# amorim-cleison/sign-language-nlp

Measured on AMD Instinct MI355X. Metric: train seq/s (batch=50,len=48), higher is better.
Workload: dtype bf16x3; 1 GPU; cfg2: Transformer train step E512 H8 N6 F512 batch 50 len 48 |src| 3000 |tgt| 202 dropout 0.1, fwd+CE+bwd+clip(0.5)+SGD(m=.9); launch=eager stream launches (auto: timed both in 9 untimed pre-warmup steps + warmup), per_gpu=independent fit (grid shard)

## Files before the change

### sign-language-nlp_amd/csrc/common.hpp

```cpp
#pragma once
#include <vector>
#include <hip/hip_runtime.h>
#include <atomic>
#include <mutex>
#include <stdint.h>
#include <stdio.h>
#include <string.h>

#include "../../include/slnlp.h"

namespace slnlp {

void set_error(const char* fmt, ...);

#define SLNLP_CHECK_ARG(cond, ...)                 \
    do {                                           \
        if (!(cond)) {                             \
            ::slnlp::set_error(__VA_ARGS__);       \
            return SLNLP_ERR_INVALID_ARG;          \
        }                                          \
    } while (0)

#define SLNLP_CHECK_LAUNCH(what)                                              \
    do {                                                                      \
        hipError_t e__ = hipGetLastError();                                   \
        if (e__ != hipSuccess) {                                              \
            ::slnlp::set_error("%s: %s", what, hipGetErrorString(e__));       \
            return SLNLP_ERR_LAUNCH;                                          \
        }                                                                     \
    } while (0)

#define SLNLP_TRY(expr)            \
    do {                           \
        int rc__ = (expr);         \
        if (rc__ != 0) return rc__; \
    } while (0)

static inline int ceil_div(long a, long b) { return (int)((a + b - 1) / b); }

struct DeviceOnce {
    std::mutex mu;
    std::atomic<bool> done[64];
    DeviceOnce() { for (auto& d : done) d.store(false, std::memory_order_relaxed); }
    template <class F>
    int run(F&& init) {
        int dev = 0;
        if (hipGetDevice(&dev) != hipSuccess || dev < 0 || dev >= 64) dev = 0;
        if (done[dev].load(std::memory_order_acquire)) return 0;
        std::lock_guard<std::mutex> lk(mu);
        if (done[dev].load(std::memory_order_relaxed)) return 0;
        const int rc = init();
        if (rc == 0) done[dev].store(true, std::memory_order_release);
        return rc;
    }
};

#ifndef SLNLP_PROBE_FENCES
#define SLNLP_PROBE_FENCES 0
#endif
__device__ __forceinline__ void probe_kernel_begin() {
#if SLNLP_PROBE_FENCES & 1
    __builtin_amdgcn_fence(__ATOMIC_ACQUIRE, "agent");
    asm volatile("s_waitcnt vmcnt(0)" ::: "memory");
#endif
}
__device__ __forceinline__ void probe_kernel_end() {
#if SLNLP_PROBE_FENCES & 2
    asm volatile("s_waitcnt vmcnt(0)" ::: "memory");
    __builtin_amdgcn_fence(__ATOMIC_RELEASE, "agent");
    asm volatile("s_waitcnt vmcnt(0)" ::: "memory");
#endif
}

__device__ __forceinline__ void gather_id_rows(const int64_t* __restrict__ X, const int64_t* __restrict__ order, long first, int B, int S,
                                               int64_t* __restrict__ out) {
    const int lane = threadIdx.x & 63;
    const int wave = __builtin_amdgcn_readfirstlane((int)(blockIdx.x * 4 + (threadIdx.x >> 6)));
    const int nwaves = gridDim.x * 4;
    for (int r = wave; r < B; r += nwaves) {
        const int64_t* src = X + (order ? order[r] : first + r) * S;
        int64_t* dst = out + (long)r * S;
        for (int c = lane; c < S; c += 64) dst[c] = src[c];
    }
}
static inline int gather_rows_grid(int B) { return B >= 256 ? 64 : (B + 3) / 4; }

template <class Row = long, class Count, class F>
__device__ __forceinline__ void wave_rows(Count n, F f) {
    const int lane = threadIdx.x & 63;
    const int wave = __builtin_amdgcn_readfirstlane((int)(blockIdx.x * 4 + (threadIdx.x >> 6)));
    const int nwaves = gridDim.x * 4;
    for (Row r = wave; r < n; r += nwaves) f(r, lane);
}
constexpr int WAVE_ROWS_MAX_BLOCKS = 2048;
static inline int wave_rows_grid(int64_t n) { return (int)((n + 3) / 4 < WAVE_ROWS_MAX_BLOCKS ? (n + 3) / 4 : WAVE_ROWS_MAX_BLOCKS); }
__device__ __forceinline__ int lanes_below(unsigned long long ballot) {
    return (int)__builtin_amdgcn_mbcnt_hi((unsigned)(ballot >> 32), __builtin_amdgcn_mbcnt_lo((unsigned)ballot, 0u));
}

struct RngState {
    unsigned long long seed;
    unsigned long long step;
};

struct DropKey { unsigned ks[5]; };
__device__ __forceinline__ DropKey dropout_key(const unsigned long long* rng, int site) {
    const unsigned long long k = rng[0] + 0x9E3779B97F4A7C15ull * rng[1];
    DropKey K;
    K.ks[0] = (unsigned)k; K.ks[1] = (unsigned)(k >> 32); K.ks[2] = (unsigned)site; K.ks[3] = 0u;
    K.ks[4] = 0x1BD11BDAu ^ K.ks[0] ^ K.ks[1] ^ K.ks[2] ^ K.ks[3];
    return K;
}

#ifndef SLNLP_THREEFRY_ROUNDS
#define SLNLP_THREEFRY_ROUNDS 12
#endif
__device__ __forceinline__ uint4 threefry4x32(unsigned c0, unsigned c1, const DropKey& K) {
    constexpr int ROT[8][2] = {{10, 26}, {11, 21}, {13, 27}, {23, 5}, {6, 20}, {17, 11}, {25, 10}, {18, 20}};
    unsigned x0 = c0 + K.ks[0], x1 = c1 + K.ks[1], x2 = K.ks[2], x3 = K.ks[3];
#pragma unroll
    for (int r = 0; r < SLNLP_THREEFRY_ROUNDS; ++r) {
        if ((r & 1) == 0) {
            x0 += x1; x1 = __builtin_rotateleft32(x1, ROT[r & 7][0]) ^ x0;
            x2 += x3; x3 = __builtin_rotateleft32(x3, ROT[r & 7][1]) ^ x2;
        } else {
            x0 += x3; x3 = __builtin_rotateleft32(x3, ROT[r & 7][0]) ^ x0;
            x2 += x1; x1 = __builtin_rotateleft32(x1, ROT[r & 7][1]) ^ x2;
        }
        if ((r & 3) == 3) {
            const int s = (r + 1) >> 2;
            x0 += K.ks[s % 5]; x1 += K.ks[(s + 1) % 5]; x2 += K.ks[(s + 2) % 5]; x3 += K.ks[(s + 3) % 5] + (unsigned)s;
        }
    }
    return make_uint4(x0, x1, x2, x3);
}

constexpr unsigned SEED_STAGE_BOOTSTRAP = SLNLP_BOOT_STAGE;
struct SeedKey { unsigned ks[5]; unsigned epoch; };
__device__ __forceinline__ SeedKey seed_key(unsigned long long seed, unsigned epoch) {
    SeedKey K;
    K.ks[0] = (unsigned)seed; K.ks[1] = (unsigned)(seed >> 32); K.ks[2] = 0u; K.ks[3] = 0u;
    K.ks[4] = 0x1BD11BDAu ^ K.ks[0] ^ K.ks[1];
    K.epoch = epoch;
    return K;
}
__device__ __forceinline__ uint4 seed_words(unsigned index, unsigned word2, const SeedKey& K) {
    constexpr int ROT[8][2] = {{10, 26}, {11, 21}, {13, 27}, {23, 5}, {6, 20}, {17, 11}, {25, 10}, {18, 20}};
    unsigned x0 = index + K.ks[0], x1 = K.epoch + K.ks[1], x2 = word2 + K.ks[2], x3 = K.ks[3];
#pragma unroll
    for (int r = 0; r < SLNLP_THREEFRY_ROUNDS; ++r) {
        if ((r & 1) == 0) {
            x0 += x1; x1 = __builtin_rotateleft32(x1, ROT[r & 7][0]) ^ x0;
            x2 += x3; x3 = __builtin_rotateleft32(x3, ROT[r & 7][1]) ^ x2;
        } else {
            x0 += x3; x3 = __builtin_rotateleft32(x3, ROT[r & 7][0]) ^ x0;
            x2 += x1; x1 = __builtin_rotateleft32(x1, ROT[r & 7][1]) ^ x2;
        }
        if ((r & 3) == 3) {
            const int s = (r + 1) >> 2;
            x0 += K.ks[s % 5]; x1 += K.ks[(s + 1) % 5]; x2 += K.ks[(s + 2) % 5]; x3 += K.ks[(s + 3) % 5] + (unsigned)s;
        }
    }
    return make_uint4(x0, x1, x2, x3);
}

__device__ __forceinline__ unsigned drop_cc(unsigned c) { return ((c >> 5) << 4) | (c & 15u); }
__device__ __forceinline__ int drop_half(unsigned c) { return (int)((c >> 4) & 1u); }

__device__ __forceinline__ uint4 dropout_bits8(const DropKey& key, unsigned r4, unsigned cc) { return threefry4x32(cc, r4, key); }

__host__ __device__ __forceinline__ unsigned dropout_threshold(float p) {
    const double t = (double)p * 65536.0 + 0.5;
    return t >= 65535.0 ? 65535u : (unsigned)t;
}

__device__ __forceinline__ unsigned pick_lot(const uint4& v, int half, int r) {
    const unsigned long long lo = (unsigned long long)v.x | ((unsigned long long)v.y << 32);
    const unsigned long long hi = (unsigned long long)v.z | ((unsigned long long)v.w << 32);
    return (unsigned)((half ? hi : lo) >> (16 * (r & 3))) & 0xFFFFu;
}

__device__ __forceinline__ bool dropout_keep(const DropKey& key, unsigned r, unsigned c, unsigned thr) {
    const uint4 b = dropout_bits8(key, r >> 2, drop_cc(c));
    return pick_lot(b, drop_half(c), (int)(r & 3u)) >= thr;
}
__device__ __forceinline__ bool dropout_keep(const unsigned long long* rng, int site,
                                             unsigned r, unsigned c, unsigned thr) {
    return dropout_keep(dropout_key(rng, site), r, c, thr);
}

struct PlaneOut {
    unsigned short* hi = nullptr;
    unsigned short* lo = nullptr;
    unsigned char* q8 = nullptr;
};
__device__ __forceinline__ unsigned pack_fp8x4(float a, float b, float c, float d) {
    a = fminf(fmaxf(a, -448.f), 448.f); b = fminf(fmaxf(b, -448.f), 448.f);
    c = fminf(fmaxf(c, -448.f), 448.f); d = fminf(fmaxf(d, -448.f), 448.f);
    int w = __builtin_amdgcn_cvt_pk_fp8_f32(a, b, 0, false);
    w = __builtin_amdgcn_cvt_pk_fp8_f32(c, d, w, true);
    return (unsigned)w;
}
__device__ __forceinline__ void split_bf16(float x, unsigned short& h, unsigned short& l) {
    const __bf16 hb = (__bf16)x;
    h = __builtin_bit_cast(unsigned short, hb);
    const __bf16 b = (__bf16)(x - (float)hb);
    l = __builtin_bit_cast(unsigned short, b);
}
__device__ __forceinline__ unsigned short head_bf16(float x) { return __builtin_bit_cast(unsigned short, (__bf16)x); }
__device__ __forceinline__ void store_planes1(const PlaneOut& po, long idx, float v) {
    if (!po.hi) return;
    unsigned short h, l;
    split_bf16(v, h, l);
    po.hi[idx] = h;
    po.lo[idx] = l;
    if (po.q8) po.q8[idx] = (unsigned char)(pack_fp8x4(v, 0.f, 0.f, 0.f) & 0xFFu);
}
__device__ __forceinline__ void store_planes4(const PlaneOut& po, long idx, float4 v) {
    if (!po.hi) return;
    unsigned short h[4], l[4];
    split_bf16(v.x, h[0], l[0]); split_bf16(v.y, h[1], l[1]); split_bf16(v.z, h[2], l[2]); split_bf16(v.w, h[3], l[3]);
    uint2 w;
    w.x = h[0] | ((unsigned)h[1] << 16); w.y = h[2] | ((unsigned)h[3] << 16);
    *reinterpret_cast<uint2*>(po.hi + idx) = w;
    w.x = l[0] | ((unsigned)l[1] << 16); w.y = l[2] | ((unsigned)l[3] << 16);
    *reinterpret_cast<uint2*>(po.lo + idx) = w;
    if (po.q8) *reinterpret_cast<unsigned*>(po.q8 + idx) = pack_fp8x4(v.x, v.y, v.z, v.w);
}

template <int CTRL>
__device__ __forceinline__ float dpp_mov(float v) {
    return __builtin_bit_cast(float, __builtin_amdgcn_update_dpp(0, __builtin_bit_cast(int, v), CTRL, 0xF, 0xF, true));
}
constexpr int DPP_XOR1 = 0xB1, DPP_XOR2 = 0x4E;
constexpr int DPP_HALF_MIRROR = 0x141, DPP_MIRROR = 0x140;
__device__ __forceinline__ float lane_bcast(float v, int lane) {
    return __builtin_bit_cast(float, __builtin_amdgcn_readlane(__builtin_bit_cast(int, v), lane));
}
__device__ __forceinline__ float row16_sum(float v) {
    v += dpp_mov<DPP_XOR1>(v);
    v += dpp_mov<DPP_XOR2>(v);
    v += dpp_mov<DPP_HALF_MIRROR>(v);
    v += dpp_mov<DPP_MIRROR>(v);
    return v;
}
__device__ __forceinline__ float row16_max(float v) {
    v = fmaxf(v, dpp_mov<DPP_XOR1>(v));
    v = fmaxf(v, dpp_mov<DPP_XOR2>(v));
    v = fmaxf(v, dpp_mov<DPP_HALF_MIRROR>(v));
    v = fmaxf(v, dpp_mov<DPP_MIRROR>(v));
    return v;
}
__device__ __forceinline__ float wave_sum(float v) {
    v = row16_sum(v);
    return (lane_bcast(v, 0) + lane_bcast(v, 16)) + (lane_bcast(v, 32) + lane_bcast(v, 48));
}
__device__ __forceinline__ float wave_max(float v) {
    v = row16_max(v);
    return fmaxf(fmaxf(lane_bcast(v, 0), lane_bcast(v, 16)), fmaxf(lane_bcast(v, 32), lane_bcast(v, 48)));
}
template <int CTRL>
__device__ __forceinline__ double dpp_mov_d(double v) {
    const int lo = __builtin_amdgcn_update_dpp(0, __double2loint(v), CTRL, 0xF, 0xF, true);
    const int hi = __builtin_amdgcn_update_dpp(0, __double2hiint(v), CTRL, 0xF, 0xF, true);
    return __hiloint2double(hi, lo);
// ... 264 lines not shown
```

### sign-language-nlp_amd/csrc/gemm_planes.hip

```cpp
#include <algorithm>
#include <vector>

#include "common.hpp"
#include "gemm_jobs.hpp"

namespace slnlp {

typedef __attribute__((ext_vector_type(8))) __bf16 bf16x8;
typedef __attribute__((ext_vector_type(4))) short s16x4;
typedef __attribute__((ext_vector_type(8))) short s16x8;
typedef __attribute__((ext_vector_type(4))) float f32x4;
typedef __attribute__((address_space(3))) void* lds_vp;
typedef __attribute__((address_space(1))) const void* glb_vp;
typedef __attribute__((ext_vector_type(4))) unsigned int u32x4;

constexpr int PT = 64;
constexpr int PTHREADS = 512;

__device__ __forceinline__ int mswz(int k) { return (((k >> 1) & 1) | (((k >> 3) & 1) << 1)) << 1; }

template <bool KMAJOR>
__device__ __forceinline__ int img_off(int row, int k) {
    if (KMAJOR) return row * PT + ((((k >> 3) ^ (row & 7)) << 3) | (k & 7));
    return k * PT + ((((row >> 3) ^ mswz(k)) << 3) | (row & 7));
}

template <bool KMAJOR>
__device__ __forceinline__ unsigned plane_lane_off(long ld, int row0, int wave, int lane) {
    const int line = 8 * wave + (lane >> 3), ps = lane & 7;
    const long e = KMAJOR ? (long)(row0 + line) * ld + ((ps ^ (line & 7)) << 3) : (long)line * ld + row0 + ((ps ^ mswz(line)) << 3);
    return (unsigned)(e * 2);
}
__device__ __forceinline__ void dma_piece(const unsigned short* __restrict__ plane, long kterm, unsigned lane_off, unsigned short* dst) {
    const char* src = reinterpret_cast<const char*>(plane + kterm) + lane_off;
    __builtin_amdgcn_global_load_lds((glb_vp)src, (lds_vp)dst, 16, 0, 0);
}

template <bool KMAJOR>
__device__ __forceinline__ bf16x8 pfrag(const unsigned short* __restrict__ img, int r0, int kk, int lane) {
    if (KMAJOR) {
        return *reinterpret_cast<const bf16x8*>(img + img_off<true>(r0 + (lane & 15), kk * 32 + ((lane >> 4) << 3)));
    } else {
        const int i = lane & 15, kb = kk * 32 + ((lane >> 4) << 3) + (i >> 2), col = r0 + ((i & 3) << 2);
        typedef __attribute__((address_space(3))) s16x4* lds_p;
        const s16x4 v0 = __builtin_amdgcn_ds_read_tr16_b64_v4i16((lds_p)(img + img_off<false>(col, kb)));
        const s16x4 v1 = __builtin_amdgcn_ds_read_tr16_b64_v4i16((lds_p)(img + img_off<false>(col, kb + 4)));
        const s16x8 v = {v0[0], v0[1], v0[2], v0[3], v1[0], v1[1], v1[2], v1[3]};
        return __builtin_bit_cast(bf16x8, v);
    }
}

template <bool KMAJOR>
__device__ __forceinline__ int img32_off(int row, int k) {
    if (KMAJOR) {
        const int line = row >> 1, sl = ((row & 1) << 2) | (k >> 3);
        return line * PT + (((sl ^ (line & 7)) << 3) | (k & 7));
    }
    return img_off<false>(row, k);
}
template <bool KMAJOR>
__device__ __forceinline__ unsigned slab32_lane_off(long ld, int row0, int row_last, int wave, int lane) {
    const int h = wave >> 2, line = 8 * (wave & 3) + (lane >> 3), ps = lane & 7;
    const int r_img = min(row0 + PT * h, row_last);
    long e;
    if (KMAJOR) {
        const int sl = ps ^ (line & 7);
        e = (long)(r_img + 2 * line + (sl >> 2)) * ld + ((sl & 3) << 3);
    } else {
        e = (long)line * ld + r_img + ((ps ^ mswz(line)) << 3);
    }
    return (unsigned)(e * 2);
}
template <bool KMAJOR>
__device__ __forceinline__ bf16x8 pfrag32(const unsigned short* __restrict__ img, int r0, int lane) {
    if (KMAJOR) return *reinterpret_cast<const bf16x8*>(img + img32_off<true>(r0 + (lane & 15), (lane >> 4) << 3));
    return pfrag<false>(img, r0, 0, lane);
}

__device__ __forceinline__ float pbf2f(unsigned short h) { return __uint_as_float(((unsigned)h) << 16); }

__device__ __forceinline__ void st_agent2(float* p, float a, float b) {
    const unsigned long long v = (unsigned long long)__float_as_uint(a) | ((unsigned long long)__float_as_uint(b) << 32);
    __hip_atomic_store(reinterpret_cast<unsigned long long*>(p), v, __ATOMIC_RELAXED, __HIP_MEMORY_SCOPE_AGENT);
}
__device__ __forceinline__ float2 ld_agent2(const float* p) {
    const unsigned long long v = __hip_atomic_load(reinterpret_cast<const unsigned long long*>(p), __ATOMIC_RELAXED, __HIP_MEMORY_SCOPE_AGENT);
    return make_float2(__uint_as_float((unsigned)v), __uint_as_float((unsigned)(v >> 32)));
}

#if SLNLP_PROBE_FENCES == 128
constexpr int TS_MAX = 1 << 16;
constexpr int TS_W = 8;
__device__ unsigned long long g_ts[TS_MAX][TS_W];
__device__ unsigned g_ts_n;
#ifdef SLNLP_PROBE_EPI
#define TS_CLK(slot) do { } while (0)
#else
#define TS_CLK(slot) do { if (slot == 1) ts[6] = __builtin_amdgcn_s_memtime(); if (slot == 2) ts[7] = __builtin_amdgcn_s_memtime(); } while (0)
#endif
#define TS_MARK(slot) do { if (threadIdx.x == 0) { ts[slot] = __builtin_amdgcn_s_memrealtime(); \
        TS_CLK(slot); } } while (0)
#else
#define TS_MARK(slot) do { } while (0)
#endif
#if SLNLP_PROBE_FENCES == 128 && defined(SLNLP_PROBE_EPI)
#define TS_EPI(slot) do { if (threadIdx.x == 0) ts[slot] = __builtin_amdgcn_s_memrealtime(); } while (0)
#else
#define TS_EPI(slot) do { } while (0)
#endif

template <int BM, int BN>
struct WaveGrid {
    static constexpr int WN = BM % 64 == 0 ? 2 : 4, WM = 8 / WN, WN_SH = WN == 2 ? 1 : 2;
    static constexpr int MT = BM / WM / 16, NT = BN / WN / 16;
    static constexpr int SUBM = (BM + PT - 1) / PT;
    static_assert(BM % (16 * WM) == 0 && BN % (16 * WN) == 0, "whole MFMA tiles per wave");
    static __device__ __forceinline__ int wm0(int wave) { return (wave >> WN_SH) * (BM / WM); }
    static __device__ __forceinline__ int wn0(int wave) { return (wave & (WN - 1)) * (BN / WN); }
};

__device__ __forceinline__ unsigned plane_lane_off_clamped(long ld, int row0, int row_max, int wave, int lane) {
    const int line = 8 * wave + (lane >> 3), ps = lane & 7;
    return (unsigned)(((long)min(row0 + line, row_max) * ld + ((ps ^ (line & 7)) << 3)) * 2);
}

template <int NSPLIT, bool AK, bool BK, int BM, int BN, int BKS, int NST>
__device__ __forceinline__ void plane_kloop(const slnlp_gemm_args& g, unsigned short* smem, int bm0, int bn0, int kt0, int kt1,
                                            bool do_rowsum, f32x4 (&acc)[WaveGrid<BM, BN>::MT][WaveGrid<BM, BN>::NT],
                                            float (&rowsum)[WaveGrid<BM, BN>::SUBM], unsigned long long* ts) {
    constexpr int NPA = NSPLIT == 3 ? 2 : 1, NPB = NSPLIT >= 2 ? 2 : 1;
    using WG = WaveGrid<BM, BN>;
    constexpr int SUBM = WG::SUBM, SUBN = BN / PT;
    constexpr int MT = WG::MT, NT = WG::NT;
    constexpr int IMG_E = PT * BKS;
    constexpr int A_E = BM * BKS, B_E = BN * BKS;
    constexpr int A_LO = A_E, B_HI = NPA * A_E, B_LO = B_HI + B_E;
    constexpr int STAGE = NPA * A_E + NPB * B_E;
    constexpr bool HALF_A = BM % PT != 0;
    constexpr int PIECES = HALF_A ? NPA + 1 + NPB * SUBN : (NPA * SUBM + NPB * SUBN) * BKS / 64;
    constexpr int PIECES_HI = HALF_A && NPA == 1 ? PIECES - 1 : PIECES;
    static_assert(BKS == 64 || (BM % 128 == 0 && BN % 128 == 0), "32-k stages move 128-row slabs");
    static_assert(!HALF_A || (AK && BKS == 64 && BM == PT + PT / 2), "the 96-row panel is built for k-major A and 64-k stages");
    const int tid = threadIdx.x, lane = tid & 63, wave = __builtin_amdgcn_readfirstlane(tid >> 6);
    const int wm0 = WG::wm0(wave), wn0 = WG::wn0(wave);
    const int am_last = ((g.M + PT - 1) / PT - 1) * PT, bn_last = ((g.N + PT - 1) / PT - 1) * PT;

    constexpr int APC = HALF_A ? 1 : BKS == 64 ? SUBM : SUBM / 2, BPC = BKS == 64 ? SUBN : SUBN / 2;
    unsigned aoff[APC], boff[BPC];
    unsigned aoff_half = 0;
#pragma unroll
    for (int q = 0; q < APC; ++q) {
        if constexpr (HALF_A) aoff[q] = plane_lane_off_clamped(g.lda_p, bm0, am_last + PT - 1, wave, lane);
        else if constexpr (BKS == 64) aoff[q] = plane_lane_off<AK>(g.lda_p, BM > PT ? min(bm0 + q * PT, am_last) : bm0, wave, lane);
        else aoff[q] = slab32_lane_off<AK>(g.lda_p, bm0 + 2 * q * PT, am_last, wave, lane);
    }
    if constexpr (HALF_A) aoff_half = plane_lane_off_clamped(g.lda_p, bm0 + PT, am_last + PT - 1, wave & 3, lane);
#pragma unroll
    for (int q = 0; q < BPC; ++q) {
        if constexpr (BKS == 64) boff[q] = plane_lane_off<BK>(g.ldb_p, BN > PT ? min(bn0 + q * PT, bn_last) : bn0, wave, lane);
        else boff[q] = slab32_lane_off<BK>(g.ldb_p, bn0 + 2 * q * PT, bn_last, wave, lane);
    }
    constexpr int PSTEP = BKS == 64 ? 1 : 2;
    auto issue = [&](int kt, int stage) {
        const int k0 = (kt < kt1 ? kt : kt0) * BKS;
        const long ka = AK ? (long)k0 : (long)k0 * g.lda_p, kb = BK ? (long)k0 : (long)k0 * g.ldb_p;
        unsigned short* s = smem + stage * STAGE + wave * 512;
#pragma unroll
        for (int q = 0; q < APC; ++q) {
            dma_piece(g.A_hi, ka, aoff[q], s + q * PSTEP * IMG_E);
            if (NPA == 2) dma_piece(g.A_lo, ka, aoff[q], s + (A_LO + q * PSTEP * IMG_E));
        }
        if constexpr (HALF_A) {
            unsigned short* sh = smem + stage * STAGE + IMG_E + (wave & 3) * 512;
            if (wave < 4) dma_piece(g.A_hi, ka, aoff_half, sh);
            else if (NPA == 2) dma_piece(g.A_lo, ka, aoff_half, sh + A_LO);
        }
#pragma unroll
        for (int q = 0; q < BPC; ++q) {
            dma_piece(g.B_hi, kb, boff[q], s + (B_HI + q * PSTEP * IMG_E));
            if (NPB == 2) dma_piece(g.B_lo, kb, boff[q], s + (B_LO + q * PSTEP * IMG_E));
        }
    };

    for (int t = 0; t < NST - 1; ++t) issue(kt0 + t, t);
    for (int kt = kt0; kt < kt1; ++kt) {
        const int it = kt - kt0;
        if (PIECES_HI == PIECES || wave < 4) asm volatile("s_waitcnt vmcnt(%0)\n\ts_waitcnt lgkmcnt(0)" ::"n"((NST - 2) * PIECES) : "memory");
        else asm volatile("s_waitcnt vmcnt(%0)\n\ts_waitcnt lgkmcnt(0)" ::"n"((NST - 2) * PIECES_HI) : "memory");
        __builtin_amdgcn_s_barrier();
        asm volatile("" ::: "memory");
#if SLNLP_PROBE_FENCES == 128
        if (kt == kt0) TS_MARK(1);
#endif
        issue(kt + NST - 1, (it + NST - 1) % NST);
        const unsigned short* s = smem + (it % NST) * STAGE;
#pragma unroll
        for (int kk = 0; kk < BKS / 32; ++kk) {
            constexpr int JB = NT > 4 ? 4 : NT;
            bf16x8 ah[MT], al[MT];
#pragma unroll
            for (int i = 0; i < MT; ++i) {
                const int row = wm0 + 16 * i;
                if constexpr (BKS == 64) {
                    ah[i] = pfrag<AK>(s + (row / PT) * IMG_E, row % PT, kk, lane);
                    if (NPA == 2) al[i] = pfrag<AK>(s + (A_LO + (row / PT) * IMG_E), row % PT, kk, lane);
                } else {
                    ah[i] = pfrag32<AK>(s + (row / PT) * IMG_E, row % PT, lane);
                    if (NPA == 2) al[i] = pfrag32<AK>(s + (A_LO + (row / PT) * IMG_E), row % PT, lane);
                }
            }
#pragma unroll
            for (int j0 = 0; j0 < NT; j0 += JB) {
                bf16x8 bh[JB], bl[JB];
#pragma unroll
                for (int j = 0; j < JB; ++j) {
                    const int row = wn0 + 16 * (j0 + j);
                    if constexpr (BKS == 64) {
                        bh[j] = pfrag<BK>(s + (B_HI + (row / PT) * IMG_E), row % PT, kk, lane);
                        if (NPB == 2) bl[j] = pfrag<BK>(s + (B_LO + (row / PT) * IMG_E), row % PT, kk, lane);
                    } else {
                        bh[j] = pfrag32<BK>(s + (B_HI + (row / PT) * IMG_E), row % PT, lane);
                        if (NPB == 2) bl[j] = pfrag32<BK>(s + (B_LO + (row / PT) * IMG_E), row % PT, lane);
                    }
                }
#pragma unroll
                for (int i = 0; i < MT; ++i)
#pragma unroll
                    for (int j = 0; j < JB; ++j) {
                        f32x4& c = acc[i][j0 + j];
                        if (NPA == 2) c = __builtin_amdgcn_mfma_f32_16x16x32_bf16(al[i], bh[j], c, 0, 0, 0);
                        if (NPB == 2) c = __builtin_amdgcn_mfma_f32_16x16x32_bf16(ah[i], bl[j], c, 0, 0, 0);
                        c = __builtin_amdgcn_mfma_f32_16x16x32_bf16(ah[i], bh[j], c, 0, 0, 0);
                    }
            }
        }
        if (do_rowsum) {
            constexpr int OCT = BKS / 8;
            const int row = tid & 63, kq = ((tid >> 6) % OCT) * 8, sub0 = (tid >> 6) / OCT;
#pragma unroll
            for (int sm = 0; sm < SUBM; sm += 8 / OCT) {
                const int im = sm + sub0;
                if constexpr (HALF_A) {
                    if (im * PT + row >= BM) continue;
                }
                float t = 0.f;
#pragma unroll
                for (int k = 0; k < 8; ++k) {
                    const int off = BKS == 64 ? img_off<AK>(row, kq + k) : img32_off<AK>(row, kq + k);
                    t += pbf2f(s[im * IMG_E + off]);
                    if (NPA == 2) t += pbf2f(s[A_LO + im * IMG_E + off]);
                }
                if (BKS == 64) rowsum[sm] += t;
                else if (kt & 1) rowsum[sm + 1] += t;
                else rowsum[sm] += t;
            }
        }
    }
}

template <int NSPLIT, int BM, int BN, int BKS, int NST>
__device__ __forceinline__ void plane_tile(const PlaneJob& job, int lid, bool placed, unsigned short* smem) {
    unsigned long long* tsp = nullptr;
#if SLNLP_PROBE_FENCES == 128
    unsigned long long ts[TS_W] = {0, 0, 0, 0, 0, 0, 0, 0};
    struct TsFlush {
        unsigned long long* t;
        __device__ ~TsFlush() {
            if (threadIdx.x == 0) {
                t[4] = __builtin_amdgcn_s_memrealtime();
                unsigned hw;
                asm volatile("s_getreg_b32 %0, hwreg(HW_REG_XCC_ID)" : "=s"(hw));
                t[5] = ((unsigned long long)hw << 32) | blockIdx.x;
                const unsigned i = atomicAdd(&g_ts_n, 1u) & (unsigned)(TS_MAX - 1);
                for (int k = 0; k < TS_W; ++k) g_ts[i][k] = t[k];
            }
        }
    } ts_flush{ts};
    tsp = ts;
    TS_MARK(0);
#endif
    using WG = WaveGrid<BM, BN>;
    constexpr int SUBM = WG::SUBM;
    constexpr int MT = WG::MT, NT = WG::NT;
    constexpr int KSUB = PT / BKS;
    const slnlp_gemm_args& g = job.a;
    const int tid = threadIdx.x, lane = tid & 63, wave = __builtin_amdgcn_readfirstlane(tid >> 6);
    const int wm0 = WG::wm0(wave), wn0 = WG::wn0(wave);
    const int nks = job.nks;
    int bx, by, ks, tile;
    {
        const int nwg = job.tiles_x * job.tiles_y * nks;
        const int xcd = lid & 7, q = nwg >> 3, r = nwg & 7;
        const int t = placed ? lid : (xcd < r ? xcd * (q + 1) : r * (q + 1) + (xcd - r) * q) + (lid >> 3);
        const int ntiles = job.tiles_x * job.tiles_y;
        ks = t / ntiles;
        tile = t - ks * ntiles;
        constexpr int GR = BM >= 256 ? 2 : BM >= 128 ? 4 : 8;
        const int grp = tile / (GR * job.tiles_x), rem = tile - grp * (GR * job.tiles_x);
        const int rows_here = min(GR, job.tiles_y - grp * GR);
        bx = rem / rows_here;
        by = grp * GR + (rem - bx * rows_here);
        tile = by * job.tiles_x + bx;
    }
    const int bm0 = by * BM, bn0 = bx * BN;
    const int M = g.M, N = g.N, K = g.K;
    const int ktiles = (K + PT - 1) / PT;
    const int kt0 = (int)((long)ktiles * ks / nks) * KSUB, kt1 = (int)((long)ktiles * (ks + 1) / nks) * KSUB;

    f32x4 acc[MT][NT];
#pragma unroll
    for (int i = 0; i < MT; ++i)
#pragma unroll
        for (int j = 0; j < NT; ++j) acc[i][j] = f32x4{0.f, 0.f, 0.f, 0.f};
    const bool do_rowsum = (g.rowsum_a != nullptr) && (bx == 0);
    float rowsum[SUBM];
#pragma unroll
    for (int i = 0; i < SUBM; ++i) rowsum[i] = 0.f;

    if constexpr (BM % PT != 0) {
        if (job.variant == 0) plane_kloop<NSPLIT, true, true, BM, BN, BKS, NST>(g, smem, bm0, bn0, kt0, kt1, do_rowsum, acc, rowsum, tsp);
        else if (job.variant == 1) plane_kloop<NSPLIT, true, false, BM, BN, BKS, NST>(g, smem, bm0, bn0, kt0, kt1, do_rowsum, acc, rowsum, tsp);
        else if constexpr (NSPLIT == 3) {
            if (job.variant == 3) plane_kloop<2, true, false, BM, BN, BKS, NST + 1>(g, smem, bm0, bn0, kt0, kt1, do_rowsum, acc, rowsum, tsp);
        }
    } else {
        if (job.variant == 0) plane_kloop<NSPLIT, true, true, BM, BN, BKS, NST>(g, smem, bm0, bn0, kt0, kt1, do_rowsum, acc, rowsum, tsp);
        else if (job.variant == 1) plane_kloop<NSPLIT, true, false, BM, BN, BKS, NST>(g, smem, bm0, bn0, kt0, kt1, do_rowsum, acc, rowsum, tsp);
        else if (job.variant == 2) plane_kloop<NSPLIT, false, false, BM, BN, BKS, NST>(g, smem, bm0, bn0, kt0, kt1, do_rowsum, acc, rowsum, tsp);
        else if constexpr (NSPLIT == 3) {
            if (job.variant == 3) plane_kloop<2, true, false, BM, BN, BKS, NST + 1>(g, smem, bm0, bn0, kt0, kt1, do_rowsum, acc, rowsum, tsp);
            else plane_kloop<2, false, false, BM, BN, BKS, NST + 1>(g, smem, bm0, bn0, kt0, kt1, do_rowsum, acc, rowsum, tsp);
        }
    }
    TS_MARK(2);
    asm volatile("s_waitcnt vmcnt(0)" ::: "memory");
    __builtin_amdgcn_s_barrier();
    float* rs = reinterpret_cast<float*>(smem);
    int* flag = reinterpret_cast<int*>(smem) + SUBM * PTHREADS;
    float rs_row = 0.f;
    if (do_rowsum) {
        if (BKS == 64) {
#pragma unroll
            for (int sm = 0; sm < SUBM; ++sm) rs[(sm * 8 + (tid >> 6)) * PT + (tid & 63)] = rowsum[sm];
        } else {
#pragma unroll
            for (int sm = 0; sm < SUBM; sm += 2) {
                const int im = sm + (tid >> 8), o = (tid >> 6) & 3;
                rs[(im * 8 + o) * PT + (tid & 63)] = rowsum[sm];
                rs[(im * 8 + o + 4) * PT + (tid & 63)] = rowsum[sm + 1];
            }
        }
        __syncthreads();
        if (tid < BM) {
#pragma unroll
            for (int w = 0; w < 8; ++w) rs_row += rs[((tid / PT) * 8 + w) * PT + (tid % PT)];
        }
    }
    if (nks > 1) {
        constexpr int SC = 17;
        constexpr int TILE_FLOATS = BM * BN;
        const __amdgpu_buffer_rsrc_t mine =
            __builtin_amdgcn_make_buffer_rsrc(job.part + ((long)tile * nks + ks) * TILE_FLOATS, 0, TILE_FLOATS * 4, 0x00020000);
#pragma unroll
        for (int i = 0; i < MT; ++i)
#pragma unroll
            for (int j = 0; j < NT; ++j)
                __builtin_amdgcn_raw_buffer_store_b128(__builtin_bit_cast(u32x4, acc[i][j]), mine, tid * 16, (i * NT + j) * PTHREADS * 16, SC);
        if (do_rowsum && tid < BM)
            __hip_atomic_store(job.part_rs + ((long)by * nks + ks) * BM + tid, rs_row, __ATOMIC_RELAXED, __HIP_MEMORY_SCOPE_AGENT);
        if (job.hand_off == 4) return;
        asm volatile("s_waitcnt vmcnt(0)" ::: "memory");
        __syncthreads();
        if (tid == 0) {
            if (job.hand_off == 3) {
                __builtin_amdgcn_fence(__ATOMIC_RELEASE, "agent");
                asm volatile("s_waitcnt vmcnt(0)" ::: "memory");
            }
            const bool last = __hip_atomic_fetch_add(job.counters + tile, 1, __ATOMIC_RELAXED, __HIP_MEMORY_SCOPE_AGENT) == nks - 1;
            if (last && job.hand_off >= 2) {
                __builtin_amdgcn_fence(__ATOMIC_ACQUIRE, "agent");
                asm volatile("s_waitcnt vmcnt(0)" ::: "memory");
            }
            *flag = last;
        }
        __syncthreads();
        if (!*flag) return;
#pragma unroll
        for (int i = 0; i < MT; ++i)
#pragma unroll
            for (int j = 0; j < NT; ++j) acc[i][j] = f32x4{0.f, 0.f, 0.f, 0.f};
        rs_row = 0.f;
        constexpr int HALVES = MT * NT > 16 ? 2 : 1, MH = MT / HALVES;
#pragma unroll
        for (int half = 0; half < HALVES; ++half) {
#pragma unroll 1
            for (int s = 0; s < nks; ++s) {
                const __amdgpu_buffer_rsrc_t q =
                    __builtin_amdgcn_make_buffer_rsrc(job.part + ((long)tile * nks + s) * TILE_FLOATS, 0, TILE_FLOATS * 4, 0x00020000);
#pragma unroll
                for (int i = half * MH; i < (half + 1) * MH; ++i)
#pragma unroll
                    for (int j = 0; j < NT; ++j) {
                        const u32x4 p = __builtin_amdgcn_raw_buffer_load_b128(q, tid * 16, (i * NT + j) * PTHREADS * 16, SC);
                        acc[i][j] += __builtin_bit_cast(f32x4, p);
                    }
                if (half == 0 && do_rowsum && tid < BM)
                    rs_row += __hip_atomic_load(job.part_rs + ((long)by * nks + s) * BM + tid, __ATOMIC_RELAXED, __HIP_MEMORY_SCOPE_AGENT);
            }
        }
        if (tid == 0) __hip_atomic_store(job.counters + tile, 0, __ATOMIC_RELAXED, __HIP_MEMORY_SCOPE_AGENT);
    }
    if (do_rowsum && tid < BM && bm0 + tid < M) g.rowsum_a[bm0 + tid] = rs_row;
    TS_MARK(3);

    constexpr int SLD = BN + 4, ER = BM > 128 ? 128 : BM, ECH = BM / ER;
    const int crow = (lane >> 4) << 2, ccol = lane & 15;
    float* stg = reinterpret_cast<float*>(smem);
    float* sbias = stg + ER * SLD;
    const bool early = g.drop_p > 0.f || g.relu == 2;
    if (early && tid < BN) sbias[tid] = (g.bias && bn0 + tid < N) ? g.bias[bn0 + tid] : 0.f;
    DropKey dkey = {};
    if (g.drop_p > 0.f) dkey = dropout_key(g.rng, g.drop_site);
#pragma unroll 1
    for (int ch = 0; ch < ECH; ++ch) {
        __syncthreads();
        if (ECH == 1 || wm0 / ER == ch) {
            const int lr0 = wm0 - ch * ER + crow, lc0 = wn0 + ccol;
#pragma unroll
            for (int i = 0; i < MT; ++i)
#pragma unroll
                for (int j = 0; j < NT; ++j)
#pragma unroll
                    for (int r = 0; r < 4; ++r) stg[(lr0 + 16 * i + r) * SLD + lc0 + 16 * j] = acc[i][j][r];
#if defined(SLNLP_PROBE_EPI) && SLNLP_PROBE_EPI == 2
            if (ch == 0) TS_EPI(6);
#endif
            if constexpr (NT % 2 != 0) {
                static_assert(NT == 1, "one column tile per wave");
                if (early) {
#pragma unroll 1
                    for (int t = 0; t < MT; ++t) {
                        const int lm0 = lr0 + 16 * t, gm0 = bm0 + ch * ER + lm0, gn0 = bn0 + lc0;
                        if (gn0 >= N || gm0 >= M) continue;
                        float v[4], gt[4];
#pragma unroll
                        for (int r = 0; r < 4; ++r) {
                            v[r] = stg[(lm0 + r) * SLD + lc0];
                            gt[r] = 1.f;
                            if (g.gate && gm0 + r < M) gt[r] = g.gate[(long)(gm0 + r) * g.ldg + gn0];
                        }
                        const float bias = sbias[lc0];
                        uint4 bits = make_uint4(0, 0, 0, 0);
                        if (g.drop_p > 0.f) bits = dropout_bits8(dkey, (unsigned)gm0 >> 2, drop_cc((unsigned)gn0));
                        const int h = drop_half((unsigned)gn0);
#pragma unroll
                        for (int r = 0; r < 4; ++r) {
                            float x = v[r] + bias;
                            if (g.relu == 1) x = fmaxf(x, 0.f);
                            else if (g.relu == 2) x = tanhf(x);
                            if (g.gate) x = g.gate_mode == 1 ? x * (1.f - gt[r] * gt[r]) : (gt[r] > 0.f ? x * g.gate_scale : 0.f);
                            if (g.drop_p > 0.f) x = (pick_lot(bits, h, r) >= job.drop_thr) ? x * job.drop_scale : 0.f;
                            v[r] = x;
                        }
#pragma unroll
                        for (int r = 0; r < 4; ++r) stg[(lm0 + r) * SLD + lc0] = v[r];
                    }
                }
            } else if (early) {
                static_assert(NT % 2 == 0, "column tiles in pairs");
#pragma unroll 1
                for (int t = 0; t < MT * (NT / 2); ++t) {
                    const int lm0 = lr0 + 16 * (t / (NT / 2)), ln0 = lc0 + 32 * (t % (NT / 2));
                    const int gm0 = bm0 + ch * ER + lm0, gn0 = bn0 + ln0;
                    if (gn0 >= N || gm0 >= M) continue;
                    float v[2][4], gt[2][4];
#pragma unroll
                    for (int h = 0; h < 2; ++h)
#pragma unroll
                        for (int r = 0; r < 4; ++r) {
                            v[h][r] = stg[(lm0 + r) * SLD + ln0 + 16 * h];
                            gt[h][r] = 1.f;
                            if (g.gate && gm0 + r < M && gn0 + 16 * h < N) gt[h][r] = g.gate[(long)(gm0 + r) * g.ldg + gn0 + 16 * h];
                        }
                    const float bias[2] = {sbias[ln0], sbias[ln0 + 16]};
                    uint4 bits = make_uint4(0, 0, 0, 0);
                    if (g.drop_p > 0.f) bits = dropout_bits8(dkey, (unsigned)gm0 >> 2, drop_cc((unsigned)gn0));
#pragma unroll
                    for (int h = 0; h < 2; ++h)
#pragma unroll
                        for (int r = 0; r < 4; ++r) {
                            float x = v[h][r] + bias[h];
                            if (g.relu == 1) x = fmaxf(x, 0.f);
                            else if (g.relu == 2) x = tanhf(x);
                            if (g.gate) x = g.gate_mode == 1 ? x * (1.f - gt[h][r] * gt[h][r]) : (gt[h][r] > 0.f ? x * g.gate_scale : 0.f);
                            if (g.drop_p > 0.f) x = (pick_lot(bits, h, r) >= job.drop_thr) ? x * job.drop_scale : 0.f;
                            v[h][r] = x;
                        }
#pragma unroll
                    for (int h = 0; h < 2; ++h)
#pragma unroll
                        for (int r = 0; r < 4; ++r) stg[(lm0 + r) * SLD + ln0 + 16 * h] = v[h][r];
                }
            }
        }
#if defined(SLNLP_PROBE_EPI) && SLNLP_PROBE_EPI == 2
        if (ch == 0) TS_EPI(7);
#else
        if (ch == 0) TS_EPI(6);
#endif
        const int gmc = bm0 + ch * ER;
        const bool late_gate = !early && g.gate;
        if (job.vec_out) {
            constexpr int NPASS = ER * BN / 4 / PTHREADS, PB = NPASS > 8 ? 8 : NPASS;
            static_assert(PTHREADS % (BN / 4) == 0, "a thread keeps its four columns over the passes");
            const int c4 = (tid % (BN / 4)) << 2, gn = bn0 + c4, row0 = tid / (BN / 4);
            constexpr int RSTEP = PTHREADS / (BN / 4);
            float4 b4 = make_float4(0.f, 0.f, 0.f, 0.f);
            if (!early && g.bias && gn < N) b4 = *reinterpret_cast<const float4*>(g.bias + gn);
#pragma unroll 1
            for (int pb = 0; pb < NPASS; pb += PB) {
                float4 rr[PB], gg[PB];
#pragma unroll
                for (int pass = 0; pass < PB; ++pass) {
                    const int gm = gmc + row0 + (pb + pass) * RSTEP;
                    rr[pass] = make_float4(0.f, 0.f, 0.f, 0.f);
                    gg[pass] = make_float4(0.f, 0.f, 0.f, 0.f);
                    if (g.resid && gm < M && gn < N) rr[pass] = *reinterpret_cast<const float4*>(g.resid + (long)gm * g.ldr + gn);
                    if (late_gate && gm < M && gn < N) gg[pass] = *reinterpret_cast<const float4*>(g.gate + (long)gm * g.ldg + gn);
                }
                if (pb == 0) __syncthreads();
#if !defined(SLNLP_PROBE_EPI) || SLNLP_PROBE_EPI != 2
                if (pb == 0 && ch == 0) TS_EPI(7);
#endif
#pragma unroll
                for (int pass = 0; pass < PB; ++pass) {
                    const int row = row0 + (pb + pass) * RSTEP, gm = gmc + row;
                    if (gm >= M || gn >= N) continue;
                    float4 v = *reinterpret_cast<const float4*>(stg + row * SLD + c4);
                    if (!early) {
                        v.x += b4.x; v.y += b4.y; v.z += b4.z; v.w += b4.w;
                        if (g.relu == 1) { v.x = fmaxf(v.x, 0.f); v.y = fmaxf(v.y, 0.f); v.z = fmaxf(v.z, 0.f); v.w = fmaxf(v.w, 0.f); }
                        if (late_gate) {
                            const float4 t = gg[pass];
                            if (g.gate_mode == 1) {
                                v.x = __fmul_rn(v.x, 1.f - t.x * t.x); v.y = __fmul_rn(v.y, 1.f - t.y * t.y);
                                v.z = __fmul_rn(v.z, 1.f - t.z * t.z); v.w = __fmul_rn(v.w, 1.f - t.w * t.w);
                            } else {
                                v.x = t.x > 0.f ? __fmul_rn(v.x, g.gate_scale) : 0.f; v.y = t.y > 0.f ? __fmul_rn(v.y, g.gate_scale) : 0.f;
                                v.z = t.z > 0.f ? __fmul_rn(v.z, g.gate_scale) : 0.f; v.w = t.w > 0.f ? __fmul_rn(v.w, g.gate_scale) : 0.f;
                            }
                        }
                    }
                    if (g.resid) { v.x += rr[pass].x; v.y += rr[pass].y; v.z += rr[pass].z; v.w += rr[pass].w; }
                    if (g.C) *reinterpret_cast<float4*>(g.C + (long)gm * g.ldc + gn) = v;
                    if (g.C_hi) {
                        PlaneOut po;
                        po.hi = g.C_hi;
                        po.lo = g.C_lo;
                        if (g.C_lo) store_planes4(po, (long)gm * g.ldc_p + gn, v);
                        else {
                            uint2 w;
                            w.x = head_bf16(v.x) | ((unsigned)head_bf16(v.y) << 16);
                            w.y = head_bf16(v.z) | ((unsigned)head_bf16(v.w) << 16);
                            *reinterpret_cast<uint2*>(g.C_hi + (long)gm * g.ldc_p + gn) = w;
                        }
                    }
                }
            }
        } else {
            __syncthreads();
#pragma unroll 1
            for (int e = tid; e < ER * BN; e += PTHREADS) {
                const int row = e / BN, col = e % BN, gm = gmc + row, gn = bn0 + col;
                if (gm >= M || gn >= N) continue;
                float v = stg[row * SLD + col];
                if (!early) {
                    if (g.bias) v += g.bias[gn];
                    if (g.relu == 1) v = fmaxf(v, 0.f);
                    if (g.gate) {
                        const float gt = g.gate[(long)gm * g.ldg + gn];
                        v = g.gate_mode == 1 ? __fmul_rn(v, 1.f - gt * gt) : (gt > 0.f ? __fmul_rn(v, g.gate_scale) : 0.f);
                    }
                }
                if (g.resid) v += g.resid[(long)gm * g.ldr + gn];
                if (g.C) g.C[(long)gm * g.ldc + gn] = v;
                if (g.C_hi) {
                    unsigned short h, l;
                    split_bf16(v, h, l);
                    g.C_hi[(long)gm * g.ldc_p + gn] = h;
                    if (g.C_lo) g.C_lo[(long)gm * g.ldc_p + gn] = l;
                }
            }
        }
    }
}

constexpr int Q8_BK = 128;
constexpr int Q8_IMG = PT * Q8_BK;
typedef __attribute__((ext_vector_type(8))) int i32x8;

__device__ __forceinline__ void dma_q8(const unsigned char* __restrict__ plane, long ld, int row0, int k0, unsigned char* img,
                                       int wave, int lane) {
    const int line = 8 * wave + (lane >> 3), ps = lane & 7;
    const unsigned char* src = plane + (long)(row0 + line) * ld + k0 + ((ps ^ (line & 7)) << 4);
    __builtin_amdgcn_global_load_lds((glb_vp)src, (lds_vp)(img + wave * 1024), 16, 0, 0);
}

__device__ __forceinline__ i32x8 q8_frag(const unsigned char* __restrict__ img, int r0, int lane) {
    const int row = r0 + (lane & 15), q = lane >> 4;
    const uint4 lo = *reinterpret_cast<const uint4*>(img + row * Q8_BK + (((2 * q) ^ (row & 7)) << 4));
    const uint4 hi = *reinterpret_cast<const uint4*>(img + row * Q8_BK + (((2 * q + 1) ^ (row & 7)) << 4));
    return i32x8{(int)lo.x, (int)lo.y, (int)lo.z, (int)lo.w, (int)hi.x, (int)hi.y, (int)hi.z, (int)hi.w};
}

template <int BM, int BN, int NST>
__device__ __forceinline__ void q8_tile(const PlaneJob& job, int lid, unsigned char* smem) {
    constexpr int SUBM = BM / PT, SUBN = BN / PT, MT = BM / 64, NT = BN / 32;
    constexpr int STAGE = (SUBM + SUBN) * Q8_IMG, PIECES = SUBM + SUBN;
    constexpr int E8M0_ONE = 0x7F7F7F7F;
    const slnlp_gemm_args& g = job.a;
// ... 850 lines not shown
```

Baseline: 21550 seq/s.

## Precompute dropout mask during GEMM prologue and apply NT==1 epilogue in registers

Splits plane_kloop into a prologue part that issues the first NST-1 DMA stages and a main-loop part. Between the two, NT==1 tiles generate their threefry dropout keep-bits while those loads are in flight, so the RNG work no longer sits in the epilogue. The NT==1 epilogue now applies bias, activation, gate and dropout directly on the accumulator registers instead of round-tripping through LDS, and it loads bias per lane rather than staging it in shared memory. It also forces nks=1 for the 96-row panel shape and reads the rng words through the constant address space. The cost is extra live registers (the keep mask and gate values) during the k-loop, which could reduce occupancy.

```diff
diff --git a/sign-language-nlp_amd/csrc/common.hpp b/sign-language-nlp_amd/csrc/common.hpp
--- a/sign-language-nlp_amd/csrc/common.hpp
+++ b/sign-language-nlp_amd/csrc/common.hpp
@@ -104,13 +104,14 @@
 };
 
 struct DropKey { unsigned ks[5]; };
-__device__ __forceinline__ DropKey dropout_key(const unsigned long long* rng, int site) {
-    const unsigned long long k = rng[0] + 0x9E3779B97F4A7C15ull * rng[1];
+__device__ __forceinline__ DropKey dropout_key(unsigned long long seed, unsigned long long step, int site) {
+    const unsigned long long k = seed + 0x9E3779B97F4A7C15ull * step;
     DropKey K;
     K.ks[0] = (unsigned)k; K.ks[1] = (unsigned)(k >> 32); K.ks[2] = (unsigned)site; K.ks[3] = 0u;
     K.ks[4] = 0x1BD11BDAu ^ K.ks[0] ^ K.ks[1] ^ K.ks[2] ^ K.ks[3];
     return K;
 }
+__device__ __forceinline__ DropKey dropout_key(const unsigned long long* rng, int site) { return dropout_key(rng[0], rng[1], site); }
 
 #ifndef SLNLP_THREEFRY_ROUNDS
 #define SLNLP_THREEFRY_ROUNDS 12
diff --git a/sign-language-nlp_amd/csrc/gemm_planes.hip b/sign-language-nlp_amd/csrc/gemm_planes.hip
--- a/sign-language-nlp_amd/csrc/gemm_planes.hip
+++ b/sign-language-nlp_amd/csrc/gemm_planes.hip
@@ -1,4 +1,5 @@
 #include <algorithm>
+#include <type_traits>
 #include <vector>
 
 #include "common.hpp"
@@ -124,7 +125,7 @@
     return (unsigned)(((long)min(row0 + line, row_max) * ld + ((ps ^ (line & 7)) << 3)) * 2);
 }
 
-template <int NSPLIT, bool AK, bool BK, int BM, int BN, int BKS, int NST>
+template <int NSPLIT, bool AK, bool BK, int BM, int BN, int BKS, int NST, int PART>
 __device__ __forceinline__ void plane_kloop(const slnlp_gemm_args& g, unsigned short* smem, int bm0, int bn0, int kt0, int kt1,
                                             bool do_rowsum, f32x4 (&acc)[WaveGrid<BM, BN>::MT][WaveGrid<BM, BN>::NT],
                                             float (&rowsum)[WaveGrid<BM, BN>::SUBM], unsigned long long* ts) {
@@ -182,7 +183,10 @@
         }
     };
 
-    for (int t = 0; t < NST - 1; ++t) issue(kt0 + t, t);
+    if constexpr (PART == 0) {
+        for (int t = 0; t < NST - 1; ++t) issue(kt0 + t, t);
+        return;
+    }
     for (int kt = kt0; kt < kt1; ++kt) {
         const int it = kt - kt0;
         if (PIECES_HI == PIECES || wave < 4) asm volatile("s_waitcnt vmcnt(%0)\n\ts_waitcnt lgkmcnt(0)" ::"n"((NST - 2) * PIECES) : "memory");
@@ -286,7 +290,7 @@
     const slnlp_gemm_args& g = job.a;
     const int tid = threadIdx.x, lane = tid & 63, wave = __builtin_amdgcn_readfirstlane(tid >> 6);
     const int wm0 = WG::wm0(wave), wn0 = WG::wn0(wave);
-    const int nks = job.nks;
+    const int nks = BM % PT != 0 ? 1 : job.nks;
     int bx, by, ks, tile;
     {
         const int nwg = job.tiles_x * job.tiles_y * nks;
@@ -317,21 +321,43 @@
 #pragma unroll
     for (int i = 0; i < SUBM; ++i) rowsum[i] = 0.f;
 
-    if constexpr (BM % PT != 0) {
-        if (job.variant == 0) plane_kloop<NSPLIT, true, true, BM, BN, BKS, NST>(g, smem, bm0, bn0, kt0, kt1, do_rowsum, acc, rowsum, tsp);
-        else if (job.variant == 1) plane_kloop<NSPLIT, true, false, BM, BN, BKS, NST>(g, smem, bm0, bn0, kt0, kt1, do_rowsum, acc, rowsum, tsp);
-        else if constexpr (NSPLIT == 3) {
-            if (job.variant == 3) plane_kloop<2, true, false, BM, BN, BKS, NST + 1>(g, smem, bm0, bn0, kt0, kt1, do_rowsum, acc, rowsum, tsp);
-        }
-    } else {
-        if (job.variant == 0) plane_kloop<NSPLIT, true, true, BM, BN, BKS, NST>(g, smem, bm0, bn0, kt0, kt1, do_rowsum, acc, rowsum, tsp);
-        else if (job.variant == 1) plane_kloop<NSPLIT, true, false, BM, BN, BKS, NST>(g, smem, bm0, bn0, kt0, kt1, do_rowsum, acc, rowsum, tsp);
-        else if (job.variant == 2) plane_kloop<NSPLIT, false, false, BM, BN, BKS, NST>(g, smem, bm0, bn0, kt0, kt1, do_rowsum, acc, rowsum, tsp);
-        else if constexpr (NSPLIT == 3) {
-            if (job.variant == 3) plane_kloop<2, true, false, BM, BN, BKS, NST + 1>(g, smem, bm0, bn0, kt0, kt1, do_rowsum, acc, rowsum, tsp);
-            else plane_kloop<2, false, false, BM, BN, BKS, NST + 1>(g, smem, bm0, bn0, kt0, kt1, do_rowsum, acc, rowsum, tsp);
-        }
-    }
+    auto kloop = [&](auto part) {
+        constexpr int PART = decltype(part)::value;
+        if constexpr (BM % PT != 0) {
+            if (job.variant == 0) plane_kloop<NSPLIT, true, true, BM, BN, BKS, NST, PART>(g, smem, bm0, bn0, kt0, kt1, do_rowsum, acc, rowsum, tsp);
+            else if (job.variant == 1) plane_kloop<NSPLIT, true, false, BM, BN, BKS, NST, PART>(g, smem, bm0, bn0, kt0, kt1, do_rowsum, acc, rowsum, tsp);
+            else if constexpr (NSPLIT == 3) {
+                if (job.variant == 3) plane_kloop<2, true, false, BM, BN, BKS, NST + 1, PART>(g, smem, bm0, bn0, kt0, kt1, do_rowsum, acc, rowsum, tsp);
+            }
+        } else {
+            if (job.variant == 0) plane_kloop<NSPLIT, true, true, BM, BN, BKS, NST, PART>(g, smem, bm0, bn0, kt0, kt1, do_rowsum, acc, rowsum, tsp);
+            else if (job.variant == 1) plane_kloop<NSPLIT, true, false, BM, BN, BKS, NST, PART>(g, smem, bm0, bn0, kt0, kt1, do_rowsum, acc, rowsum, tsp);
+            else if (job.variant == 2) plane_kloop<NSPLIT, false, false, BM, BN, BKS, NST, PART>(g, smem, bm0, bn0, kt0, kt1, do_rowsum, acc, rowsum, tsp);
+            else if constexpr (NSPLIT == 3) {
+                if (job.variant == 3) plane_kloop<2, true, false, BM, BN, BKS, NST + 1, PART>(g, smem, bm0, bn0, kt0, kt1, do_rowsum, acc, rowsum, tsp);
+                else plane_kloop<2, false, false, BM, BN, BKS, NST + 1, PART>(g, smem, bm0, bn0, kt0, kt1, do_rowsum, acc, rowsum, tsp);
+            }
+        }
+    };
+    kloop(std::integral_constant<int, 0>{});
+    unsigned keep = 0;
+    if constexpr (NT == 1) {
+        if (g.drop_p > 0.f) {
+            typedef const __attribute__((address_space(4))) unsigned long long* const_words;
+            const const_words rw = (const_words)g.rng;
+            const DropKey key = dropout_key(rw[0], rw[1], g.drop_site);
+            const int gn0 = bn0 + wn0 + (lane & 15), h = drop_half((unsigned)gn0);
+#pragma unroll
+            for (int i = 0; i < MT; ++i) {
+                const int gm0 = bm0 + wm0 + ((lane >> 4) << 2) + 16 * i;
+                const uint4 bits = dropout_bits8(key, (unsigned)gm0 >> 2, drop_cc((unsigned)gn0));
+#pragma unroll
+                for (int r = 0; r < 4; ++r) keep |= (pick_lot(bits, h, r) >= job.drop_thr ? 1u : 0u) << (4 * i + r);
+            }
+            asm volatile("" : "+v"(keep));
+        }
+    }
+    kloop(std::integral_constant<int, 1>{});
     TS_MARK(2);
     asm volatile("s_waitcnt vmcnt(0)" ::: "memory");
     __builtin_amdgcn_s_barrier();
@@ -418,14 +444,48 @@
     float* stg = reinterpret_cast<float*>(smem);
     float* sbias = stg + ER * SLD;
     const bool early = g.drop_p > 0.f || g.relu == 2;
-    if (early && tid < BN) sbias[tid] = (g.bias && bn0 + tid < N) ? g.bias[bn0 + tid] : 0.f;
+    float bias1 = 0.f;
+    if constexpr (NT == 1) {
+        if (early && g.bias && bn0 + wn0 + ccol < N) bias1 = g.bias[bn0 + wn0 + ccol];
+    } else {
+        if (early && tid < BN) sbias[tid] = (g.bias && bn0 + tid < N) ? g.bias[bn0 + tid] : 0.f;
+    }
     DropKey dkey = {};
-    if (g.drop_p > 0.f) dkey = dropout_key(g.rng, g.drop_site);
+    if (NT != 1 && g.drop_p > 0.f) dkey = dropout_key(g.rng, g.drop_site);
 #pragma unroll 1
     for (int ch = 0; ch < ECH; ++ch) {
         __syncthreads();
         if (ECH == 1 || wm0 / ER == ch) {
             const int lr0 = wm0 - ch * ER + crow, lc0 = wn0 + ccol;
+            if constexpr (NT == 1) {
+                static_assert(ECH == 1, "one chunk");
+                const int gn0 = bn0 + lc0;
+                if (early && gn0 < N) {
+                    float gt[MT][4];
+#pragma unroll
+                    for (int i = 0; i < MT; ++i)
+#pragma unroll
+                        for (int r = 0; r < 4; ++r) {
+                            const int gm = bm0 + lr0 + 16 * i + r;
+                            gt[i][r] = 1.f;
+                            if (g.gate && gm < M) gt[i][r] = g.gate[(long)gm * g.ldg + gn0];
+                        }
+                    auto each = [&](auto&& step) {
+#pragma unroll
+                        for (int i = 0; i < MT; ++i)
+#pragma unroll
+                            for (int r = 0; r < 4; ++r) acc[i][0][r] = step(acc[i][0][r], i, r);
+                    };
+                    each([&](float x, int, int) { return x + bias1; });
+                    if (g.relu == 1) each([&](float x, int, int) { return fmaxf(x, 0.f); });
+                    else if (g.relu == 2) each([&](float x, int, int) { return tanhf(x); });
+                    if (g.gate) {
+                        if (g.gate_mode == 1) each([&](float x, int i, int r) { return x * (1.f - gt[i][r] * gt[i][r]); });
+                        else each([&](float x, int i, int r) { return gt[i][r] > 0.f ? x * g.gate_scale : 0.f; });
+                    }
+                    if (g.drop_p > 0.f) each([&](float x, int i, int r) { return (keep >> (4 * i + r) & 1u) ? x * job.drop_scale : 0.f; });
+                }
+            }
 #pragma unroll
             for (int i = 0; i < MT; ++i)
 #pragma unroll
@@ -436,36 +496,7 @@
             if (ch == 0) TS_EPI(6);
 #endif
             if constexpr (NT % 2 != 0) {
-                static_assert(NT == 1, "one column tile per wave");
-                if (early) {
-#pragma unroll 1
-                    for (int t = 0; t < MT; ++t) {
-                        const int lm0 = lr0 + 16 * t, gm0 = bm0 + ch * ER + lm0, gn0 = bn0 + lc0;
-                        if (gn0 >= N || gm0 >= M) continue;
-                        float v[4], gt[4];
-#pragma unroll
-                        for (int r = 0; r < 4; ++r) {
-                            v[r] = stg[(lm0 + r) * SLD + lc0];
-                            gt[r] = 1.f;
-                            if (g.gate && gm0 + r < M) gt[r] = g.gate[(long)(gm0 + r) * g.ldg + gn0];
-                        }
-                        const float bias = sbias[lc0];
-                        uint4 bits = make_uint4(0, 0, 0, 0);
-                        if (g.drop_p > 0.f) bits = dropout_bits8(dkey, (unsigned)gm0 >> 2, drop_cc((unsigned)gn0));
-                        const int h = drop_half((unsigned)gn0);
-#pragma unroll
-                        for (int r = 0; r < 4; ++r) {
-                            float x = v[r] + bias;
-                            if (g.relu == 1) x = fmaxf(x, 0.f);
-                            else if (g.relu == 2) x = tanhf(x);
-                            if (g.gate) x = g.gate_mode == 1 ? x * (1.f - gt[r] * gt[r]) : (gt[r] > 0.f ? x * g.gate_scale : 0.f);
-                            if (g.drop_p > 0.f) x = (pick_lot(bits, h, r) >= job.drop_thr) ? x * job.drop_scale : 0.f;
-                            v[r] = x;
-                        }
-#pragma unroll
-                        for (int r = 0; r < 4; ++r) stg[(lm0 + r) * SLD + lc0] = v[r];
-                    }
-                }
+                static_assert(NT == 1, "one column tile per wave: phase 1b ran in registers, above");
             } else if (early) {
                 static_assert(NT % 2 == 0, "column tiles in pairs");
 #pragma unroll 1
```

Measured after the change: 21920 seq/s, median of 6. 1.02x the previous value.
